# ethz-asl/laser_slam

Hardware: NVIDIA H100
Metric: ICP registrations/s (131072-pt scan vs 524288-pt map, 30 iterations) (higher is better)
Workload: dtype f32

## Files before the change

### laser_slam_b200/csrc/ls_api.cu

```cuda
#include <cstdarg>
#include <cstddef>
#include <cstdio>
#include <cstdlib>
#include <cstring>
#include <string>
#include <utility>
#include <vector>

#include "../../include/ls_b200.h"
#include "ls_kernels.cuh"

using namespace ls;

#define LS_VERSION 100

struct Workspace {
  cudaStream_t stream = nullptr;
  cudaEvent_t ev0 = nullptr, ev1 = nullptr, ev2 = nullptr, ev_launch = nullptr;
  int n_cap = 0, m_cap = 0, cells_cap = 0, tab_cap = 0, hist_cap = 0;
  BuildArrays A{};
  BuildState* bs = nullptr;
  float4* rd = nullptr;
  int* pos = nullptr;
  float4 *vq = nullptr, *vpts = nullptr;
// ... 318 lines not shown
  hp.lists.vq = w->vq;
  hp.lists.vpts = w->vpts;
  hp.lists.n = n;
  hp.work = w->work;
  hp.shard_rank = 0;
  hp.shard_count = 1;
  std::memset(&hp.link, 0, sizeof(hp.link));
  hp.T_hist = want_hist ? w->T_hist : nullptr;
  if (want_hist) {
    CU(cudaMemsetAsync(w->T_hist, 0, (size_t)prm->max_iterations * 16 * sizeof(float), w->stream));
    w->stream_dirty = true;
  }
  hp.want_matches = want_matches ? 1 : 0;
  hp.phase_ns = nullptr;
  std::memcpy(hp.T0, T0, sizeof(hp.T0));
  return LS_OK;
}

int prep_icp(ls_ctx* ctx, Workspace* w, const ls_icp_params* prm, const float4* reading_dev, int n, const float T0[16],
             bool want_matches, bool want_hist) {
  w->job_host->reading = reading_dev;
  w->job_host->n = n;
  CU(cudaMemcpyAsync(w->job_dev, w->job_host, sizeof(BuildJob), cudaMemcpyHostToDevice, w->stream));
  int rc;
  if ((rc = launch_reading_sort(ctx, w->job_dev, 1, n, resolve(prm), w->stream))) return rc;
  CU(cudaEventRecord(w->ev1, w->stream));
  CU(cudaMemsetAsync(w->work, 0, sizeof(IcpWork), w->stream));
  return fill_problem(ctx, w, prm, n, T0, want_matches, want_hist);
}

int launch_icp(ls_ctx* ctx, const ls_icp_params* prm, int batch, int n_max, bool sharded = false) {
  Workspace* w0 = ctx->ws[0];
  for (int b = 0; b < batch; ++b) ctx->probs_host[b] = ctx->ws[b]->hp;
  CU(cudaMemcpyAsync(ctx->probs_dev, ctx->probs_host, sizeof(IcpProblem) * (size_t)batch, cudaMemcpyHostToDevice, w0->stream));
  IcpParamsDev dp;
  dp.max_iterations = prm->max_iterations;
  dp.trim_ratio = prm->trim_ratio;
  dp.use_differential = prm->use_differential;
  dp.min_diff_rot = prm->min_diff_rot;
  dp.min_diff_trans = prm->min_diff_trans;
  dp.smooth_length = prm->smooth_length;
  int ctas = ctx->icp_ctas / batch;
  const int need = (n_max + 31) / 32;
  if (ctas > need) ctas = need;
  if (ctas < 1) ctas = 1;
  const IcpProblem* probs = ctx->probs_dev;
  int dynamic = batch > 1 ? 1 : 0;
  void* args[] = {(void*)&probs, (void*)&ctas, (void*)&dp, (void*)&dynamic};
  if (sharded) {
    shard_slice_kernel<<<1, 32, 0, w0->stream>>>(ctx->probs_dev, w0->job_dev, w0->hp.shard_rank, w0->hp.shard_count);
    LAUNCH_CHECK();
  }
  CU(cudaEventRecord(w0->ev_launch, w0->stream));
  CU(cudaLaunchCooperativeKernel((void*)icp_kernel, dim3(ctas * batch), dim3(kIcpThreads), args, kIcpPairBytes, w0->stream));
  ++ctx->launches;
  CU(cudaEventRecord(w0->ev2, w0->stream));
  for (int b = 0; b < batch; ++b) {
    Workspace* w = ctx->ws[b];
    constexpr size_t off = offsetof(IcpWork, T_out);
    CU(cudaMemcpyAsync(reinterpret_cast<char*>(w->h_work) + off, reinterpret_cast<const char*>(w->work) + off,
                       sizeof(IcpWork) - off, cudaMemcpyDeviceToHost, w0->stream));
    CU(cudaMemcpyAsync(w->h_grid, &w->bs->grid, sizeof(Grid), cudaMemcpyDeviceToHost, w0->stream));
  }
  return LS_OK;
}

int fetch_icp(ls_ctx* ctx, Workspace* w, int n, const float T0[16], float T_out[16], ls_icp_stats* stats,
              bool batch_timing = false) {
  const IcpWork& wk = *w->h_work;
  std::memcpy(T_out, wk.T_out, 16 * sizeof(float));
  if (stats) {
    std::memset(stats, 0, sizeof(*stats));
    stats->iterations = wk.iterations;
    stats->converged = wk.converged;
    stats->max_iter_reached = wk.max_iter_reached;
    stats->last_kept = wk.last_kept;
    stats->last_limit = wk.last_limit;
    stats->used_ratio = n > 0 ? (float)wk.last_kept / (float)n : 0.f;
    float ms = 0.f, bms = 0.f, kms = 0.f;
    const Workspace* tw = batch_timing ? ctx->ws[0] : w;
    cudaEventElapsedTime(&ms, tw->ev0, ctx->ws[0]->ev2);
    cudaEventElapsedTime(&bms, tw->ev0, tw->ev1);
    cudaEventElapsedTime(&kms, ctx->ws[0]->ev_launch, ctx->ws[0]->ev2);
    stats->device_ms = ms;
    stats->build_ms = bms;
    stats->icp_ms = kms;
    stats->grid_cells = w->h_grid->n_cells0;
    stats->grid_tables = w->h_grid->n_tab1;
    stats->grid_overflow = w->h_grid->overflow;
  }
  if (wk.status != 0) {
    std::memcpy(T_out, T0, 16 * sizeof(float));
    return fail(ctx, LS_ERR_CONVERGENCE, "ICP: no point to minimise / non-finite transformation");
  }
  return LS_OK;
}

int run_icp(ls_ctx* ctx, const ls_icp_params* prm, const float4* reading_dev, int n, const float T0[16],
            float T_out[16], ls_icp_stats* stats, int32_t* opt_ids, float* opt_d2, float* opt_T_hist) {
  Workspace* w = ctx->ws[0];
  int rc;
  if ((rc = prep_icp(ctx, w, prm, reading_dev, n, T0, opt_ids || opt_d2, opt_T_hist != nullptr))) return rc;
  if ((rc = launch_icp(ctx, prm, 1, n))) return rc;
  if (opt_ids) CU(cudaMemcpyAsync(opt_ids, w->ids, (size_t)n * sizeof(int), cudaMemcpyDeviceToHost, w->stream));
  if (opt_d2) CU(cudaMemcpyAsync(opt_d2, w->d2_out, (size_t)n * sizeof(float), cudaMemcpyDeviceToHost, w->stream));
  if (opt_T_hist)
    CU(cudaMemcpyAsync(opt_T_hist, w->T_hist, (size_t)prm->max_iterations * 16 * sizeof(float), cudaMemcpyDeviceToHost,
// ... 58 lines not shown
            cudaEventCreate(&w->ev0) == cudaSuccess && cudaEventCreate(&w->ev1) == cudaSuccess &&
            cudaEventCreate(&w->ev2) == cudaSuccess && cudaEventCreate(&w->ev_launch) == cudaSuccess &&
            cudaMalloc((void**)&w->bs, sizeof(BuildState)) == cudaSuccess &&
            cudaMallocHost((void**)&w->h_work, sizeof(IcpWork)) == cudaSuccess &&
            cudaMallocHost((void**)&w->h_grid, sizeof(Grid)) == cudaSuccess;
  if (!ok) return nullptr;
  return w;
}
void free_workspace(Workspace* w) {
  if (!w) return;
  if (w->stream) cudaStreamSynchronize(w->stream);
  void* bufs[] = {w->A.sub_pts, w->A.sub_nrm, w->A.srt_pts, w->A.srt_nrm, w->A.pkey, w->A.top, w->A.cnt0, w->A.tab1, w->A.cnt1,
                  w->A.tab1_cell, w->A.pyr, w->A.topmask, w->bs, w->rd, w->pos, w->d2,
                  w->ids, w->vq, w->vpts, w->T_hist, w->d2_out, w->A.qkey, w->A.qperm, w->A.rd_s,
                  w->A.qtab_local, w->A.qtab_total, w->A.qtop_start};
  for (void* b : bufs)
    if (b) cudaFree(b);
  if (w->h_work) cudaFreeHost(w->h_work);
  if (w->h_grid) cudaFreeHost(w->h_grid);
  if (w->ev0) cudaEventDestroy(w->ev0);
  if (w->ev1) cudaEventDestroy(w->ev1);
  if (w->ev2) cudaEventDestroy(w->ev2);
  if (w->ev_launch) cudaEventDestroy(w->ev_launch);
  if (w->stream) cudaStreamDestroy(w->stream);
  delete w;
}
int ensure_workspaces(ls_ctx* ctx, int count) {
  while ((int)ctx->ws.size() < count) {
    Workspace* w = new_workspace(ctx, (int)ctx->ws.size());
    if (!w) return fail(ctx, LS_ERR_NOMEM, "workspace allocation failed");
    ctx->ws.push_back(w);
  }
  return LS_OK;
}
}

int ls_b200_init(int device, ls_ctx** out) {
  if (!out) return LS_ERR_ARG;
  *out = nullptr;
  int count = 0;
  if (cudaGetDeviceCount(&count) != cudaSuccess || count <= 0) return LS_ERR_CUDA;
  if (device < 0 || device >= count) return LS_ERR_ARG;
  ls_ctx* ctx = new ls_ctx();
  ctx->device = device;
  auto bail = [&](int code) {
    ls_b200_destroy(ctx);
    return code;
  };
  if (cudaSetDevice(device) != cudaSuccess) return bail(LS_ERR_CUDA);
  cudaDeviceProp prop;
  if (cudaGetDeviceProperties(&prop, device) != cudaSuccess) return bail(LS_ERR_CUDA);
  if (!prop.cooperativeLaunch) return bail(LS_ERR_CUDA);
  ctx->sm_count = prop.multiProcessorCount;
  int occ = 0;
  if (cudaFuncSetAttribute(icp_kernel, cudaFuncAttributeMaxDynamicSharedMemorySize, kIcpPairBytes) != cudaSuccess ||
      cudaOccupancyMaxActiveBlocksPerMultiprocessor(&occ, icp_kernel, kIcpThreads, kIcpPairBytes) != cudaSuccess || occ < 1)
    return bail(LS_ERR_CUDA);
  ctx->icp_ctas = ctx->icp_ctas_max = occ * ctx->sm_count;
  if (cudaMalloc((void**)&ctx->probs_dev, sizeof(IcpProblem) * kMaxBatch) != cudaSuccess) return bail(LS_ERR_NOMEM);
  if (cudaMallocHost((void**)&ctx->probs_host, sizeof(IcpProblem) * kMaxBatch) != cudaSuccess) return bail(LS_ERR_NOMEM);
  if (cudaMalloc((void**)&ctx->jobs_dev, sizeof(BuildJob) * kMaxBatch) != cudaSuccess) return bail(LS_ERR_NOMEM);
  if (cudaMallocHost((void**)&ctx->jobs_host, sizeof(BuildJob) * kMaxBatch) != cudaSuccess) return bail(LS_ERR_NOMEM);
  if (cudaMalloc((void**)&ctx->work_pool, sizeof(IcpWork) * kMaxBatch) != cudaSuccess) return bail(LS_ERR_NOMEM);
  if (cudaMalloc((void**)&ctx->T0_dev, 16 * sizeof(float)) != cudaSuccess) return bail(LS_ERR_NOMEM);
  if (ensure_workspaces(ctx, 1) != LS_OK) return bail(LS_ERR_NOMEM);
  *out = ctx;
  return LS_OK;
}

void ls_b200_destroy(ls_ctx* ctx) {
  if (!ctx) return;
  cudaSetDevice(ctx->device);
  for (Workspace* w : ctx->ws) free_workspace(w);
  if (ctx->probs_dev) cudaFree(ctx->probs_dev);
  if (ctx->probs_host) cudaFreeHost(ctx->probs_host);
  if (ctx->jobs_dev) cudaFree(ctx->jobs_dev);
  if (ctx->jobs_host) cudaFreeHost(ctx->jobs_host);
  if (ctx->work_pool) cudaFree(ctx->work_pool);
  void* stage[] = {ctx->reading, ctx->ref_stage, ctx->ref_nrm_stage, ctx->nrm_raw, ctx->T0_dev};
  for (void* b : stage)
    if (b) cudaFree(b);
  ls_shard_exchange_close(ctx);
  delete ctx;
}

const char* ls_b200_last_error(const ls_ctx* ctx) { return ctx ? ctx->err.c_str() : "null context"; }
uint64_t ls_b200_launch_count(const ls_ctx* ctx) { return ctx ? ctx->launches : 0; }
int ls_b200_set_icp_cta_budget(ls_ctx* ctx, int ctas) {
  if (!ctx || ctas < 0) return LS_ERR_ARG;
  BUSY_CHECK(ctx);
  ctx->icp_ctas = (ctas == 0 || ctas > ctx->icp_ctas_max) ? ctx->icp_ctas_max : ctas;
  return LS_OK;
}
int ls_b200_icp_cta_budget(const ls_ctx* ctx) { return ctx ? ctx->icp_ctas : LS_ERR_ARG; }

void ls_icp_default_params(ls_icp_params* p) {
  if (!p) return;
  p->max_iterations = 40;
  p->trim_ratio = 0.75f;
  p->use_differential = 1;
  p->min_diff_rot = 0.001f;
  p->min_diff_trans = 0.01f;
  p->smooth_length = 4;
  p->cell_size = 0.f;
  p->leaf_split = 0;
  p->max_cells = 0;
  p->reading_sampling_prob = 1.0f;
  p->reference_normals_knn = 0;
  p->reference_sampling_ratio = 1.0f;
  p->unapplied_modules = 0;
// ... 626 lines not shown
```

### laser_slam_b200/csrc/ls_grid.cuh

```cuda
#pragma once
#include <cfloat>
#include <climits>
#include <cstring>

#include <vector_types.h>
#include <vector_functions.h>

#include "ls_math.cuh"

#define LS_FB 8
#define LS_FB3 (LS_FB * LS_FB * LS_FB)

namespace ls {

struct Entry {
  uint32_t start;
  int32_t meta;
};

struct Grid {
  float org[3];
  float H0, H1;
  float inv0, inv1;
  int dim[3];
// ... 38 lines not shown
  float d[LS_KNN_MAX];
  int id[LS_KNN_MAX];
  int k;
  float cap;
  LS_HD void reset(int kk) {
    k = kk;
    cap = INFINITY;
    for (int j = 0; j < LS_KNN_MAX; ++j) { d[j] = INFINITY; id[j] = INT_MAX; }
  }
  LS_HD float bound() const { return fminf(d[k - 1], cap); }
  LS_HD void offer(float dist, int i, int) {
    if (dist > cap || !(dist < d[k - 1] || (dist == d[k - 1] && i < id[k - 1]))) return;
    for (int j = 0; j < k; ++j)
      if (id[j] == i) return;
    int j = k - 1;
    while (j > 0 && (dist < d[j - 1] || (dist == d[j - 1] && i < id[j - 1]))) {
      d[j] = d[j - 1];
      id[j] = id[j - 1];
      --j;
    }
    d[j] = dist;
    id[j] = i;
  }
  LS_HD void offer_pt(float dist, const float4& c, int p);
};

#if defined(LS_SIM_COUNTERS) && !defined(__CUDA_ARCH__)
extern thread_local long long ls_sim_cand, ls_sim_entries, ls_sim_steps;
#define LS_CNT_CAND() (++ls_sim_cand)
#define LS_CNT_ENTRY() (++ls_sim_entries)
#define LS_CNT_STEP() (++ls_sim_steps)
#else
#define LS_CNT_CAND() ((void)0)
#define LS_CNT_ENTRY() ((void)0)
#define LS_CNT_STEP() ((void)0)
#endif

#if defined(__CUDA_ARCH__)
LS_HD float4 ld_pt(const float4* p) { return __ldg(p); }
LS_HD Entry ld_entry(const Entry* e) {
  const int2 v = __ldg(reinterpret_cast<const int2*>(e));
  Entry r;
  r.start = (uint32_t)v.x;
  r.meta = v.y;
  return r;
}
LS_HD int f2i(float f) { return __float_as_int(f); }
LS_HD float i2f(int i) { return __int_as_float(i); }
LS_HD float4 ld_state4(const float4* p) { return __ldcg(p); }
LS_HD void st_state4(float4* p, const float4 v) { __stcg(p, v); }
LS_HD unsigned long long ld_mask(const unsigned long long* p) { return __ldg(p); }
LS_HD unsigned long long ld_rows(const unsigned long long* p) { return __ldg(p); }
LS_HD int ctz64(unsigned long long m) { return __ffsll((long long)m) - 1; }
#else
LS_HD float4 ld_pt(const float4* p) { LS_CNT_CAND(); return *p; }
LS_HD Entry ld_entry(const Entry* e) { LS_CNT_ENTRY(); return *e; }
LS_HD int f2i(float f) { int i; std::memcpy(&i, &f, 4); return i; }
LS_HD float i2f(int i) { float f; std::memcpy(&f, &i, 4); return f; }
LS_HD float4 ld_state4(const float4* p) { return *p; }
LS_HD void st_state4(float4* p, const float4 v) { *p = v; }
LS_HD unsigned long long ld_mask(const unsigned long long* p) { LS_CNT_ENTRY(); return *p; }
LS_HD unsigned long long ld_rows(const unsigned long long* p) { return *p; }
LS_HD int ctz64(unsigned long long m) { return __builtin_ctzll(m); }
#endif

LS_HD int coord_top(float v, float o, float inv, int n) {
  float t = floorf((v - o) * inv);
  t = fminf(fmaxf(t, 0.0f), (float)(n - 1));
  return (int)t;
}
LS_HD int coord_sub(float v, float lo, float inv) {
  float t = floorf((v - lo) * inv);
  t = fminf(fmaxf(t, 0.0f), (float)(LS_FB - 1));
  return (int)t;
}
LS_HD float cell_lo(float o, int c, float H) { return o + (float)c * H; }

LS_HD float gap(float q, float lo, float hi, float m) {
  const float a = (lo - m) - q;
  const float b = q - (hi + m);
  return fmaxf(0.0f, fmaxf(a, b));
}

#define LS_SHRINK 0.999999f

LS_HD float ball_radius(float best_d2, float margin) { return sqrtf(best_d2) * 1.000001f + margin; }

LS_HD void Best::offer_pt(float d, const float4& c, int p) { offer(d, f2i(c.w), p); }
LS_HD void TopK::offer_pt(float dist, const float4& c, int p) { offer(dist, f2i(c.w), p); }
template <class Acc>
LS_HD void consider_pt(const float4 p, int pos, float qx, float qy, float qz, Acc& b) {
  b.offer_pt(dist2(qx, qy, qz, p.x, p.y, p.z), p, pos);
}
template <class Acc>
LS_HD void consider(const float4* pts, int pos, float qx, float qy, float qz, Acc& b) {
  consider_pt(ld_pt(pts + pos), pos, qx, qy, qz, b);
}

template <class Acc>
LS_HD void scan_range(const float4* pts, uint32_t a, uint32_t e, float qx, float qy, float qz, Acc& b) {
  uint32_t pos = a;
  for (; pos + 4 <= e; pos += 4) {
    LS_CNT_STEP();
    const float4 p0 = ld_pt(pts + pos), p1 = ld_pt(pts + pos + 1), p2 = ld_pt(pts + pos + 2), p3 = ld_pt(pts + pos + 3);
    consider_pt(p0, (int)pos, qx, qy, qz, b);
    consider_pt(p1, (int)pos + 1, qx, qy, qz, b);
    consider_pt(p2, (int)pos + 2, qx, qy, qz, b);
    consider_pt(p3, (int)pos + 3, qx, qy, qz, b);
  }
  if (pos < e) LS_CNT_STEP();
  for (; pos < e; ++pos) consider(pts, (int)pos, qx, qy, qz, b);
}

template <class Acc>
LS_HD void visit_fine(const Grid& g, const Entry* tab, unsigned long long rows, float lox, float loy, float loz,
                      const float4* pts, float qx, float qy, float qz, Acc& b) {
// ... 178 lines not shown
#ifndef LS_VL_GATE
#define LS_VL_GATE 1.0f
#endif
struct VLists {
  float4* vq;
  float4* vpts;
  int n;
};

struct Collector {
  float r2;
  int cnt;
  float4* out;
  int stride;
  LS_HD float bound() const { return r2; }
  LS_HD void offer_pt(float d, const float4& c, int p) {
    if (d <= r2) {
      if (cnt < LS_VK) st_state4(out + (size_t)cnt * stride, make_float4(c.x, c.y, c.z, i2f(p)));
      else r2 = -1.0f;
      ++cnt;
    }
  }
};

LS_HD bool vlist_query(const VLists& L, const float4* pts, int i, const float4 v, const float4 c0, float qx, float qy,
                       float qz, float cap_d2, Best& b, float4& cbest) {
  const unsigned int bits = (unsigned int)f2i(v.w);
  if (bits == 0u) return false;
  const int cnt = (int)(bits & 15u);
  const float Rv = i2f((int)(bits & ~15u));
  const float Rc = Rv * 0.999996f - sqrtf(dist2(qx, qy, qz, v.x, v.y, v.z)) * 1.000004f;
  if (!(Rc > 0.0f)) return false;
  b.d2 = cap_d2;
  b.idx = INT_MAX;
  b.pos = -1;
  for (int k = 0; k < cnt; ++k) {
    const float4 c = k == 0 ? c0 : ld_state4(L.vpts + (size_t)k * L.n + i);
    const float d = dist2(qx, qy, qz, c.x, c.y, c.z);
    const int cpos = f2i(c.w);
    if (d < b.d2) {
      b.d2 = d;
      b.pos = cpos;
      cbest = c;
    } else if (d == b.d2) {
      if (b.pos < 0 || f2i(ld_pt(pts + cpos).w) < f2i(ld_pt(pts + b.pos).w)) {
        b.pos = cpos;
        cbest = c;
      }
    }
  }
  return b.d2 * 1.00001f <= Rc * Rc;
}

LS_HD void vlist_build(const Grid& g, const GridView& v, const VLists& L, int i, float qx, float qy, float qz, bool found,
                       float found_d2, float cap_d2, float motion) {
  float Rv;
  if (found) {
    const float want = sqrtf(found_d2);
    const float margin = fmaxf(want * LS_VL_REL, LS_VL_ABS) + 1e-4f;
    if (!(motion * LS_VL_GATE <= margin)) return;
    Rv = want + fminf(margin, fmaxf(0.002f, LS_VL_SKIN * motion));
  } else {
    const float want = sqrtf(cap_d2);
    if (!(motion <= want * 0.125f)) return;
    Rv = want * 1.05f + fminf(want * 0.25f, fmaxf(0.002f, 4.0f * motion));
  }
  if (!(Rv < 3.0e38f)) return;
  Collector c;
  c.r2 = Rv * Rv;
  c.cnt = 0;
  c.out = L.vpts + i;
  c.stride = L.n;
  ball_query(g, v, qx, qy, qz, c);
  float4 head = make_float4(qx, qy, qz, 0.0f);
  if (c.cnt <= LS_VK) head.w = i2f((int)((((unsigned int)f2i(Rv * 0.9999999f)) & ~15u) | (unsigned int)c.cnt));
  st_state4(L.vq + i, head);
}

LS_HDN void knn_search(const Grid& g, const GridView& v, float qx, float qy, float qz, int k, TopK& t) {
  t.reset(k);
  if (g.m <= 0) return;
  const float extent = g.H0 * (float)(g.dim[0] + g.dim[1] + g.dim[2]) + 1.0f;
  float R = g.H1;
  for (int round = 0; round < 64; ++round) {
    t.cap = R * R;
    ball_query(g, v, qx, qy, qz, t);
    if (t.d[k - 1] <= t.cap) break;
    if (R > extent + fabsf(qx - g.org[0]) + fabsf(qy - g.org[1]) + fabsf(qz - g.org[2])) break;
    R = R * 2.0f;
  }
}

LS_HD int top_index(const Grid& g, float x, float y, float z) {
  const int cx = coord_top(x, g.org[0], g.inv0, g.dim[0]);
  const int cy = coord_top(y, g.org[1], g.inv0, g.dim[1]);
  const int cz = coord_top(z, g.org[2], g.inv0, g.dim[2]);
  return (cz * g.dim[1] + cy) * g.dim[0] + cx;
}
LS_HD void top_origin(const Grid& g, int c0, float& lox, float& loy, float& loz) {
  const int cx = c0 % g.dim[0];
  const int cy = (c0 / g.dim[0]) % g.dim[1];
  const int cz = c0 / (g.dim[0] * g.dim[1]);
  lox = cell_lo(g.org[0], cx, g.H0);
  loy = cell_lo(g.org[1], cy, g.H0);
  loz = cell_lo(g.org[2], cz, g.H0);
}
LS_HD int sub_index(float x, float y, float z, float lox, float loy, float loz, float inv) {
  return (coord_sub(z, loz, inv) * LS_FB + coord_sub(y, loy, inv)) * LS_FB + coord_sub(x, lox, inv);
}

LS_HDN void grid_setup(Grid& g, const float* lo, const float* hi, float cell_size, int max_cells, int leaf_split,
                       int m) {
  float H = cell_size > 0.f ? cell_size : 2.0f;
  float ext[3], emax = 0.f, oabs = 0.f;
  for (int a = 0; a < 3; ++a) {
    ext[a] = hi[a] - lo[a];
    if (!(ext[a] >= 0.f)) ext[a] = 0.f;
    emax = fmaxf(emax, ext[a]);
    oabs = fmaxf(oabs, fmaxf(fabsf(lo[a]), fabsf(hi[a])));
  }
  for (int it = 0; it < 40; ++it) {
    double cells = 1.0;
    for (int a = 0; a < 3; ++a) cells *= floor((double)ext[a] / (double)H) + 1.0;
    if (cells <= (double)max_cells) break;
    H = H * 2.0f;
  }
  g.H0 = H;
  g.H1 = H / (float)LS_FB;
  g.inv0 = 1.0f / g.H0;
  g.inv1 = 1.0f / g.H1;
  int n = 1;
  for (int a = 0; a < 3; ++a) {
    g.org[a] = lo[a];
    int d = (int)floorf(ext[a] * g.inv0) + 1;
    if (d < 1) d = 1;
    g.dim[a] = d;
    n *= d;
  }
  g.n_cells0 = n;
  g.margin = (oabs + emax + H) * 1.9073486328125e-06f;
  g.m = m;
  g.leaf_split = leaf_split > 0 ? leaf_split : 32;
  g.n_tab1 = 0;
  g.overflow = 0;
// ... 15 lines not shown
```

### laser_slam_b200/csrc/ls_kernels.cuh

```cuda
#pragma once
#include <cuda_runtime.h>
#include <cooperative_groups.h>

#include "ls_grid.cuh"

namespace ls {

constexpr int kMaxParts = 16;
constexpr int kScanTile = 4096;
constexpr int kScanThreads = 512;
constexpr int kIcpThreads = 512;
constexpr int kIcpCtasPerSm = 1024 / kIcpThreads;
constexpr int kMaxSmooth = 15;
constexpr uint32_t kTag1 = 1u << 31, kKeyMask = (1u << 31) - 1u;

struct Parts {
  int n_parts;
  int offset[kMaxParts + 1];
  const float4* pts[kMaxParts];
  const float4* nrm[kMaxParts];
  float T[kMaxParts][16];
  int identity[kMaxParts];
};

// ... 957 lines not shown

__device__ __forceinline__ void push_pairs(const IcpProblem& P, PairQueue& Q, int sign, float sx, float sy, float sz,
                                           const float4 q, int pos) {
  const unsigned int m = __ballot_sync(0xffffffffu, sign != 0);
  if (m == 0u) return;
  if (sign) {
    float f[6], e;
    residual_terms(sx, sy, sz, q, __ldg(P.nrm + pos), f, e);
    const int slot = (Q.head + Q.cnt + __popc(m & ((1u << (threadIdx.x & 31)) - 1u))) & (kPairSlots - 1);
    float4* r = reinterpret_cast<float4*>(Q.recs + slot * 8);
    r[0] = make_float4(f[0], f[1], f[2], f[3]);
    r[1] = make_float4(f[4], f[5], e, (float)sign);
  }
  Q.cnt += __popc(m);
  __syncwarp();
  if (Q.cnt >= 32) {
    Q.acc = consume_pairs(Q.recs, Q.head, 32, Q.acc);
    Q.head = (Q.head + 32) & (kPairSlots - 1);
    Q.cnt -= 32;
    __syncwarp();
  }
}

__device__ __forceinline__ void drain_pairs(PairQueue& Q, unsigned long long* slab) {
  if (Q.cnt > 0) {
    Q.acc = consume_pairs(Q.recs, Q.head, Q.cnt, Q.acc);
    Q.head = (Q.head + Q.cnt) & (kPairSlots - 1);
    Q.cnt = 0;
  }
  const int lane = threadIdx.x & 31;
  if (lane < 28) slab[lane] = (unsigned long long)Q.acc;
  Q.acc = 0ll;
  __syncwarp();
}

__device__ __noinline__ void phase_a_search(const Grid* gp, const IcpProblem* Pp, const float* T_iter, const float* T_prev,
                                            int i, float cap, SelHists* H, unsigned int pred_bin1, unsigned int pred_pref12) {
  if (i < 0) return;
  const Grid& g = *gp;
  const IcpProblem& P = *Pp;
  const float4 r = __ldg(P.rd + i);
  float sx, sy, sz;
  xform_point(T_iter, r.x, r.y, r.z, sx, sy, sz);
  const int warm = __ldcg(P.pos + i);
  const Best b = nn_search(g, P.view, sx, sy, sz, warm, cap);
  phase_a_record(P, i, b, H, pred_bin1, pred_pref12);
  if (T_prev) {
    float px, py, pz;
    xform_point(T_prev, r.x, r.y, r.z, px, py, pz);
    vlist_build(g, P.view, P.lists, i, sx, sy, sz, b.pos >= 0, b.d2, cap, sqrtf(dist2(sx, sy, sz, px, py, pz)));
  }
}

__device__ __forceinline__ void push_searched(const IcpProblem& P, PairQueue& Q, const float* T_iter, int j, float acc_limit) {
  if (!(acc_limit >= 0.0f)) return;
  float d = INFINITY;
  if (j >= 0) d = __ldcg(P.d2 + j);
  const bool keep = d <= acc_limit;
  if (__ballot_sync(0xffffffffu, keep) == 0u) return;
  float4 q = make_float4(0.f, 0.f, 0.f, 0.f);
  float sx = 0.f, sy = 0.f, sz = 0.f;
  int pos = -1;
  if (keep) {
    pos = __ldcg(P.pos + j);
    const float4 r = __ldg(P.rd + j);
    xform_point(T_iter, r.x, r.y, r.z, sx, sy, sz);
    q = __ldg(P.view.pts + pos);
  }
  push_pairs(P, Q, keep ? 1 : 0, sx, sy, sz, q, pos);
}

__device__ __noinline__ void final_match(const Grid* gp, const IcpProblem* Pp, const float* T, int i) {
  if (i < 0) return;
  const IcpProblem& P = *Pp;
  const float4 r = __ldg(P.rd + i);
  float sx, sy, sz;
  xform_point(T, r.x, r.y, r.z, sx, sy, sz);
  const Best b = nn_search(*gp, P.view, sx, sy, sz, __ldcg(P.pos + i), INFINITY);
  const uint32_t orig = __ldg(P.qperm + i);
  P.d2_out[orig] = b.d2;
  P.ids[orig] = b.idx;
}

__device__ __forceinline__ void flush_slabs(unsigned long long (*acc_w)[28], unsigned long long* gacc) {
  __syncthreads();
  if (threadIdx.x < 28) {
    unsigned long long t = 0ull;
#pragma unroll
    for (int w = 0; w < kIcpThreads / 32; ++w) t += acc_w[w][threadIdx.x];
    if (t != 0ull) atomicAdd(&gacc[threadIdx.x], t);
  }
  __syncthreads();
}

__device__ __forceinline__ void flush_hist(const unsigned int* hs, int nbins, unsigned int* gh) {
  for (int k = threadIdx.x; k < nbins; k += kIcpThreads) {
    const unsigned int v = hs[k];
    if (v) atomicAdd(&gh[k], v);
  }
}

__global__ void __launch_bounds__(kIcpThreads, kIcpCtasPerSm)
icp_kernel(const IcpProblem* __restrict__ probs, int ctas_per_problem, IcpParamsDev prm, int dynamic) {
  const int pi = blockIdx.x / ctas_per_problem;
  const int cta = blockIdx.x - pi * ctas_per_problem;
  const IcpProblem& P = probs[pi];
  IcpWork* W = P.work;
  const bool xg = P.shard_count > 1;
  IcpWork* X = xg ? P.link.slots + P.shard_rank : W;
  const IcpWork* S0 = xg ? P.link.slots : W;
  const int n_slots = xg ? P.shard_count : 1;
  const unsigned int G = (unsigned int)ctas_per_problem;
  unsigned int xepoch = 0;
  const int tid = threadIdx.x, lane = tid & 31;

  __shared__ Grid g;
  __shared__ float T_iter[16], T_last[16];
  __shared__ SelHists hs;
  __shared__ unsigned long long acc_w[kIcpThreads / 32][28];
  __shared__ SelectOut sel;
  __shared__ unsigned int ws[kIcpThreads / 32];
  __shared__ double qh[kMaxSmooth + 2][4];
  __shared__ double th[kMaxSmooth + 2][3];
  __shared__ int flag_stop, flag_status;
  __shared__ int miss_buf[kIcpThreads / 32][64];
  extern __shared__ __align__(16) float pair_buf[];

  if (tid == 0) {
    g = P.bs->grid;
    for (int i = 0; i < 16; ++i) T_iter[i] = (i % 5 == 0) ? 1.f : 0.f;
    quat_from_T(T_iter, qh[0]);
    th[0][0] = th[0][1] = th[0][2] = 0.0;
    flag_stop = 0;
    flag_status = 0;
  }
  __syncthreads();
  PairQueue Q;
  Q.recs = pair_buf + (tid >> 5) * (kPairSlots * 8);
  Q.head = 0;
  Q.cnt = 0;
  Q.acc = 0ll;

  const int n = P.n;
  int chunk = (n + (int)G - 1) / (int)G;
  chunk = (chunk + 31) & ~31;
  const int q_begin = min(n, cta * chunk), q_end = min(n, q_begin + chunk);

  for (int i = q_begin + tid; i < q_end; i += kIcpThreads) {
    __stcg(P.pos + i, -1);
    __stcg(P.lists.vq + i, make_float4(0.f, 0.f, 0.f, 0.f));
  }

  float cap = 0.04f;
  int redo = 0;
// ... 17 lines not shown
    __syncthreads();
    {
      const float* T_prev = iter >= 1 ? T_last : nullptr;
      int* mq = miss_buf[tid >> 5];
      int n_miss = 0;
      int next = q_begin + (tid & ~31);
      for (;;) {
        int base;
        if (dynamic) {
          unsigned int bb = 0;
          if (lane == 0) bb = atomicAdd(&W->qctr[par], 32u);
          bb = __shfl_sync(0xffffffffu, bb, 0);
          if (bb >= (unsigned int)n) break;
          base = (int)bb;
        } else {
          if (next >= q_end) break;
          base = next;
          next += kIcpThreads;
        }
        const int i = base + lane;
        bool valid = i < (dynamic ? n : q_end);
        if (redo && valid) valid = !(__ldcg(P.d2 + i) < INFINITY);
        bool hit = false;
        Best b;
        b.d2 = INFINITY; b.idx = INT_MAX; b.pos = -1;
        float4 c = make_float4(0.f, 0.f, 0.f, 0.f);
        float sx = 0.f, sy = 0.f, sz = 0.f;
        if (valid) {
          const float4 r = __ldg(P.rd + i);
          const float4 v = __ldcg(P.lists.vq + i);
          const float4 c0 = __ldcg(P.lists.vpts + i);
          xform_point(T_iter, r.x, r.y, r.z, sx, sy, sz);
          hit = vlist_query(P.lists, P.view.pts, i, v, c0, sx, sy, sz, cap, b, c);
          if (hit) phase_a_record(P, i, b, &hs, pred_bin1, pred_pref12);
        }
        push_pairs(P, Q, (hit && b.pos >= 0 && b.d2 <= acc_limit) ? 1 : 0, sx, sy, sz, c, b.pos);
        const unsigned int mm = __ballot_sync(0xffffffffu, valid && !hit);
        if (mm) {
          if (valid && !hit) mq[n_miss + __popc(mm & ((1u << lane) - 1u))] = i;
          n_miss += __popc(mm);
          __syncwarp();
          if (n_miss >= 32) {
            n_miss -= 32;
            const int j = mq[n_miss + lane];
            __syncwarp();
            phase_a_search(&g, &P, T_iter, T_prev, j, cap, &hs, pred_bin1, pred_pref12);
            push_searched(P, Q, T_iter, j, acc_limit);
          }
        }
      }
      if (n_miss > 0) {
        __syncwarp();
        const int j = lane < n_miss ? mq[lane] : -1;
        phase_a_search(&g, &P, T_iter, T_prev, j, cap, &hs, pred_bin1, pred_pref12);
        __syncwarp();
        push_searched(P, Q, T_iter, j, acc_limit);
      }
    }
    drain_pairs(Q, acc_w[tid >> 5]);
    flush_slabs(acc_w, X->acc[par]);
    flush_hist(hs.h1, 1024, X->hist[par][0]);
    if (pred_bin1 != kNoPrediction) {
      flush_hist(hs.h2, 2048, X->hist[par][3]);
      flush_hist(hs.h3, 1024, X->hist[par][4]);
    }
    {
      const int hb = kHistOff + par * 5 * 2048;
      const bool pr = pred_bin1 != kNoPrediction;
      meet(hb, 1024, hb + 3 * 2048, pr ? 2048 : 0, hb + 4 * 2048, pr ? 1024 : 0);
    }
    LS_STAMP(1);

    block_select(S0->hist[par][0], 1024, 0u, true, prm.trim_ratio, &sel, ws, n_slots);
    if (sel.total == 0u) {
      if (tid == 0) { flag_status = 1; if (cta == 0) W->fail_code = 1; }
      __syncthreads();
      break;
    }
    if (sel.bin >= 1020u) {
      if (!(cap < INFINITY)) {
        if (tid == 0) { flag_status = 1; if (cta == 0) W->fail_code = 1; }
        __syncthreads();
        break;
      }
      cap = cap < 64.0f ? cap * 4.0f : INFINITY;
      ++redo;
      meet(0, 0, 0, 0, 0, 0);
      if (cta == 0 && tid == 0) {
        X->hist[par][0][1020] = 0u;
        W->qctr[par] = 0u;
      }
      problem_barrier(&X->barrier, G, epoch);
      continue;
    }
    const unsigned int bin1 = sel.bin, rem1 = sel.rem;
    if (cta == 0) {
      unsigned int* h = &X->hist[par ^ 1][0][0];
      for (int k = tid; k < 5 * 2048; k += kIcpThreads) h[k] = 0u;
      if (tid < 32) X->acc[par ^ 1][tid] = 0ull;
    }
    if (cta == 0 && tid == 0) W->qctr[par ^ 1] = 0u;
    const bool spec2 = bin1 == pred_bin1;
    if (!spec2) {
      for (int k = tid; k < 2048; k += kIcpThreads) hs.h2[k] = 0u;
      __syncthreads();
      for (int i = q_begin + tid; i < q_end; i += kIcpThreads) {
        const unsigned int key = __float_as_uint(__ldcg(P.d2 + i));
// ... 152 lines not shown
```

Before: 901.2.

## Use cooperative lane groups for tail nearest-neighbor searches in partial warps

When a warp's leftover miss queue holds few queries (at most 8), each query is now spread across a group of 4 or 8 lanes. The lanes in a group split the grid cells, sub-cells and candidate points of the ball query and reduce the best match or verlet list with shuffles. This targets the idle lanes that the per-thread search leaves during small tail batches. The kernel is templated on this path and only used for single-problem launches. The cost is extra shuffle and scan overhead, a second kernel instance, and an occupancy taken as the minimum of the two variants.

```diff
diff --git a/laser_slam_b200/csrc/ls_api.cu b/laser_slam_b200/csrc/ls_api.cu
--- a/laser_slam_b200/csrc/ls_api.cu
+++ b/laser_slam_b200/csrc/ls_api.cu
@@ -394,7 +394,8 @@
     LAUNCH_CHECK();
   }
   CU(cudaEventRecord(w0->ev_launch, w0->stream));
-  CU(cudaLaunchCooperativeKernel((void*)icp_kernel, dim3(ctas * batch), dim3(kIcpThreads), args, kIcpPairBytes, w0->stream));
+  void* const kern = dynamic ? (void*)icp_kernel<false> : (void*)icp_kernel<true>;
+  CU(cudaLaunchCooperativeKernel(kern, dim3(ctas * batch), dim3(kIcpThreads), args, kIcpPairBytes, w0->stream));
   ++ctx->launches;
   CU(cudaEventRecord(w0->ev2, w0->stream));
   for (int b = 0; b < batch; ++b) {
@@ -559,10 +560,14 @@
   if (cudaGetDeviceProperties(&prop, device) != cudaSuccess) return bail(LS_ERR_CUDA);
   if (!prop.cooperativeLaunch) return bail(LS_ERR_CUDA);
   ctx->sm_count = prop.multiProcessorCount;
-  int occ = 0;
-  if (cudaFuncSetAttribute(icp_kernel, cudaFuncAttributeMaxDynamicSharedMemorySize, kIcpPairBytes) != cudaSuccess ||
-      cudaOccupancyMaxActiveBlocksPerMultiprocessor(&occ, icp_kernel, kIcpThreads, kIcpPairBytes) != cudaSuccess || occ < 1)
+  int occ = 0, occ1 = 0;
+  if (cudaFuncSetAttribute(icp_kernel<false>, cudaFuncAttributeMaxDynamicSharedMemorySize, kIcpPairBytes) != cudaSuccess ||
+      cudaFuncSetAttribute(icp_kernel<true>, cudaFuncAttributeMaxDynamicSharedMemorySize, kIcpPairBytes) != cudaSuccess ||
+      cudaOccupancyMaxActiveBlocksPerMultiprocessor(&occ, icp_kernel<false>, kIcpThreads, kIcpPairBytes) != cudaSuccess ||
+      cudaOccupancyMaxActiveBlocksPerMultiprocessor(&occ1, icp_kernel<true>, kIcpThreads, kIcpPairBytes) != cudaSuccess)
     return bail(LS_ERR_CUDA);
+  if (occ1 < occ) occ = occ1;
+  if (occ < 1) return bail(LS_ERR_CUDA);
   ctx->icp_ctas = ctx->icp_ctas_max = occ * ctx->sm_count;
   if (cudaMalloc((void**)&ctx->probs_dev, sizeof(IcpProblem) * kMaxBatch) != cudaSuccess) return bail(LS_ERR_NOMEM);
   if (cudaMallocHost((void**)&ctx->probs_host, sizeof(IcpProblem) * kMaxBatch) != cudaSuccess) return bail(LS_ERR_NOMEM);
diff --git a/laser_slam_b200/csrc/ls_grid.cuh b/laser_slam_b200/csrc/ls_grid.cuh
--- a/laser_slam_b200/csrc/ls_grid.cuh
+++ b/laser_slam_b200/csrc/ls_grid.cuh
@@ -114,6 +114,7 @@
 LS_HD unsigned long long ld_mask(const unsigned long long* p) { return __ldg(p); }
 LS_HD unsigned long long ld_rows(const unsigned long long* p) { return __ldg(p); }
 LS_HD int ctz64(unsigned long long m) { return __ffsll((long long)m) - 1; }
+LS_HD int popc64(unsigned long long m) { return __popcll(m); }
 #else
 LS_HD float4 ld_pt(const float4* p) { LS_CNT_CAND(); return *p; }
 LS_HD Entry ld_entry(const Entry* e) { LS_CNT_ENTRY(); return *e; }
@@ -124,6 +125,7 @@
 LS_HD unsigned long long ld_mask(const unsigned long long* p) { LS_CNT_ENTRY(); return *p; }
 LS_HD unsigned long long ld_rows(const unsigned long long* p) { return *p; }
 LS_HD int ctz64(unsigned long long m) { return __builtin_ctzll(m); }
+LS_HD int popc64(unsigned long long m) { return __builtin_popcountll(m); }
 #endif
 
 LS_HD int coord_top(float v, float o, float inv, int n) {
@@ -408,29 +410,55 @@
   return b.d2 * 1.00001f <= Rc * Rc;
 }
 
-LS_HD void vlist_build(const Grid& g, const GridView& v, const VLists& L, int i, float qx, float qy, float qz, bool found,
-                       float found_d2, float cap_d2, float motion) {
+LS_HD float vlist_radius(bool found, float found_d2, float cap_d2, float motion) {
   float Rv;
   if (found) {
     const float want = sqrtf(found_d2);
     const float margin = fmaxf(want * LS_VL_REL, LS_VL_ABS) + 1e-4f;
-    if (!(motion * LS_VL_GATE <= margin)) return;
+    if (!(motion * LS_VL_GATE <= margin)) return 0.0f;
     Rv = want + fminf(margin, fmaxf(0.002f, LS_VL_SKIN * motion));
   } else {
     const float want = sqrtf(cap_d2);
-    if (!(motion <= want * 0.125f)) return;
+    if (!(motion <= want * 0.125f)) return 0.0f;
     Rv = want * 1.05f + fminf(want * 0.25f, fmaxf(0.002f, 4.0f * motion));
   }
-  if (!(Rv < 3.0e38f)) return;
+  return Rv < 3.0e38f ? Rv : 0.0f;
+}
+
+LS_HD float4 vlist_head(float qx, float qy, float qz, float Rv, int cnt) {
+  float4 head = make_float4(qx, qy, qz, 0.0f);
+  if (cnt <= LS_VK) head.w = i2f((int)((((unsigned int)f2i(Rv * 0.9999999f)) & ~15u) | (unsigned int)cnt));
+  return head;
+}
+
+LS_HD void vlist_build(const Grid& g, const GridView& v, const VLists& L, int i, float qx, float qy, float qz, bool found,
+                       float found_d2, float cap_d2, float motion) {
+  const float Rv = vlist_radius(found, found_d2, cap_d2, motion);
+  if (!(Rv > 0.0f)) return;
   Collector c;
   c.r2 = Rv * Rv;
   c.cnt = 0;
   c.out = L.vpts + i;
   c.stride = L.n;
   ball_query(g, v, qx, qy, qz, c);
-  float4 head = make_float4(qx, qy, qz, 0.0f);
-  if (c.cnt <= LS_VK) head.w = i2f((int)((((unsigned int)f2i(Rv * 0.9999999f)) & ~15u) | (unsigned int)c.cnt));
-  st_state4(L.vq + i, head);
+  st_state4(L.vq + i, vlist_head(qx, qy, qz, Rv, c.cnt));
+}
+
+LS_HD int ball_cells(const Grid& g, float qx, float qy, float qz, float r2) {
+  const float R = ball_radius(r2, g.margin);
+  const int nx = coord_top(qx + R, g.org[0], g.inv0, g.dim[0]) - coord_top(qx - R, g.org[0], g.inv0, g.dim[0]) + 1;
+  const int ny = coord_top(qy + R, g.org[1], g.inv0, g.dim[1]) - coord_top(qy - R, g.org[1], g.inv0, g.dim[1]) + 1;
+  const int nz = coord_top(qz + R, g.org[2], g.inv0, g.dim[2]) - coord_top(qz - R, g.org[2], g.inv0, g.dim[2]) + 1;
+  return nx * ny * nz;
+}
+
+LS_HD int nth_bit64(unsigned long long m, int k) {
+  int pos = 0;
+  for (int w = 32; w >= 1; w >>= 1) {
+    const int c = popc64(m & ((1ull << w) - 1ull));
+    if (k >= c) { k -= c; m >>= w; pos += w; }
+  }
+  return pos;
 }
 
 LS_HDN void knn_search(const Grid& g, const GridView& v, float qx, float qy, float qz, int k, TopK& t) {
@@ -446,6 +474,169 @@
     R = R * 2.0f;
   }
 }
+
+#if defined(__CUDACC__)
+template <int L>
+__device__ __forceinline__ int group_scan(int v, int& total) {
+  const int l = threadIdx.x & (L - 1);
+  int s = v;
+#pragma unroll
+  for (int o = 1; o < L; o <<= 1) {
+    const int t = __shfl_up_sync(0xffffffffu, s, o, L);
+    if (l >= o) s += t;
+  }
+  total = __shfl_sync(0xffffffffu, s, L - 1, L);
+  return s - v;
+}
+template <int L>
+__device__ __forceinline__ int group_owner(int off, int t) {
+  int o = 0;
+#pragma unroll
+  for (int s = L / 2; s >= 1; s >>= 1)
+    if (__shfl_sync(0xffffffffu, off, o + s, L) <= t) o += s;
+  return o;
+}
+
+template <int L, class Acc>
+__device__ __forceinline__ void group_ball(const Grid& g, const GridView& v, bool on, float qx, float qy, float qz, Acc& a) {
+  const int l = threadIdx.x & (L - 1);
+  const float R = ball_radius(a.bound(), g.margin);
+  const int x0 = coord_top(qx - R, g.org[0], g.inv0, g.dim[0]), nx = coord_top(qx + R, g.org[0], g.inv0, g.dim[0]) - x0 + 1;
+  const int y0 = coord_top(qy - R, g.org[1], g.inv0, g.dim[1]), ny = coord_top(qy + R, g.org[1], g.inv0, g.dim[1]) - y0 + 1;
+  const int z0 = coord_top(qz - R, g.org[2], g.inv0, g.dim[2]), nz = coord_top(qz + R, g.org[2], g.inv0, g.dim[2]) - z0 + 1;
+  const int n_cell = on ? nx * ny * nz : 0;
+  const int cell_rounds = __reduce_max_sync(0xffffffffu, n_cell);
+  for (int cb = 0; cb < cell_rounds; cb += L) {
+    const int c = cb + l;
+    Entry e{0u, 0};
+    unsigned long long rows = 0ull;
+    float cy = 0.f, cz = 0.f;
+    int fx = 0;
+    int n_item = 0;
+    if (c < n_cell) {
+      const int x = x0 + c % nx, y = y0 + (c / nx) % ny, z = z0 + c / (nx * ny);
+      const float cx = cell_lo(g.org[0], x, g.H0);
+      cy = cell_lo(g.org[1], y, g.H0);
+      cz = cell_lo(g.org[2], z, g.H0);
+      const float gz = gap(qz, cz, cell_lo(g.org[2], z + 1, g.H0), g.margin);
+      const float gy = gap(qy, cy, cell_lo(g.org[1], y + 1, g.H0), g.margin);
+      const float gx = gap(qx, cx, cell_lo(g.org[0], x + 1, g.H0), g.margin);
+      const float lb = gx * gx + (gy * gy + gz * gz);
+      if (!(lb * LS_SHRINK > a.bound())) {
+        const size_t ci = ((size_t)z * g.dim[1] + y) * g.dim[0] + x;
+        e = ld_entry(v.top + ci);
+        rows = ld_rows(v.topmask + ci);
+        if (e.meta > 0) {
+          n_item = 1;
+        } else if (e.meta < 0) {
+          const float R1 = ball_radius(a.bound(), g.margin);
+          fx = coord_sub(qx - R1, cx, g.inv1) | coord_sub(qx + R1, cx, g.inv1) << 8;
+          const int fy0 = coord_sub(qy - R1, cy, g.inv1), fy1 = coord_sub(qy + R1, cy, g.inv1);
+          const int fz0 = coord_sub(qz - R1, cz, g.inv1), fz1 = coord_sub(qz + R1, cz, g.inv1);
+          const unsigned long long ym = (unsigned long long)((2u << fy1) - (1u << fy0));
+          unsigned long long in = 0ull;
+          for (int zz = fz0; zz <= fz1; ++zz) in |= ym << (zz * LS_FB);
+          rows &= in;
+          n_item = popc64(rows);
+        }
+      }
+    }
+    int n_items;
+    const int ioff = group_scan<L>(n_item, n_items);
+    const int item_rounds = __reduce_max_sync(0xffffffffu, n_items);
+    for (int ib = 0; ib < item_rounds; ib += L) {
+      const int t = ib + l;
+      const int o = group_owner<L>(ioff, t);
+      const int k = t - __shfl_sync(0xffffffffu, ioff, o, L);
+      const uint32_t o_start = __shfl_sync(0xffffffffu, e.start, o, L);
+      const int o_meta = __shfl_sync(0xffffffffu, e.meta, o, L);
+      const unsigned long long o_rows =
+          (unsigned long long)__shfl_sync(0xffffffffu, (unsigned int)rows, o, L) |
+          (unsigned long long)__shfl_sync(0xffffffffu, (unsigned int)(rows >> 32), o, L) << 32;
+      const float o_cy = __shfl_sync(0xffffffffu, cy, o, L), o_cz = __shfl_sync(0xffffffffu, cz, o, L);
+      const int o_fx = __shfl_sync(0xffffffffu, fx, o, L);
+      uint32_t r0 = 0u, r1 = 0u;
+      if (t < n_items) {
+        if (o_meta > 0) {
+          r0 = o_start;
+          r1 = o_start + (uint32_t)o_meta;
+        } else {
+          const int bit = nth_bit64(o_rows, k);
+          const int z = bit / LS_FB, y = bit % LS_FB;
+          const float gz = gap(qz, cell_lo(o_cz, z, g.H1), cell_lo(o_cz, z + 1, g.H1), g.margin);
+          const float gy = gap(qy, cell_lo(o_cy, y, g.H1), cell_lo(o_cy, y + 1, g.H1), g.margin);
+          const float lb = gy * gy + gz * gz;
+          if (!(lb * LS_SHRINK > a.bound())) {
+            const Entry* row = v.tab1 + (size_t)(~o_meta) * LS_FB3 + (z * LS_FB + y) * LS_FB;
+            const Entry e0 = ld_entry(row + (o_fx & 255));
+            const Entry e1 = ld_entry(row + (o_fx >> 8));
+            r0 = e0.start;
+            r1 = e1.start + (uint32_t)e1.meta;
+          }
+        }
+      }
+      int n_cand;
+      const int coff = group_scan<L>((int)(r1 - r0), n_cand);
+      const int cand_rounds = __reduce_max_sync(0xffffffffu, n_cand);
+      for (int kb = 0; kb < cand_rounds; kb += 4 * L) {
+        int p[4];
+#pragma unroll
+        for (int u = 0; u < 4; ++u) {
+          const int tt = kb + u * L + l;
+          const int oo = group_owner<L>(coff, tt);
+          const int at = (int)__shfl_sync(0xffffffffu, r0, oo, L) + (tt - __shfl_sync(0xffffffffu, coff, oo, L));
+          p[u] = tt < n_cand ? at : -1;
+        }
+        float4 pt[4];
+#pragma unroll
+        for (int u = 0; u < 4; ++u) pt[u] = p[u] >= 0 ? ld_pt(v.pts + p[u]) : make_float4(0.f, 0.f, 0.f, 0.f);
+#pragma unroll
+        for (int u = 0; u < 4; ++u) a.offer(p[u] >= 0, dist2(qx, qy, qz, pt[u].x, pt[u].y, pt[u].z), pt[u], p[u]);
+        a.sync();
+      }
+    }
+  }
+}
+
+template <int L>
+struct GroupBest {
+  Best b;
+  __device__ float bound() const { return b.d2; }
+  __device__ void offer(bool take, float d, const float4& c, int p) {
+    if (take) b.offer_pt(d, c, p);
+  }
+  __device__ void sync() {
+#pragma unroll
+    for (int o = 1; o < L; o <<= 1) {
+      const float d = __shfl_xor_sync(0xffffffffu, b.d2, o, L);
+      const int i = __shfl_xor_sync(0xffffffffu, b.idx, o, L);
+      const int p = __shfl_xor_sync(0xffffffffu, b.pos, o, L);
+      b.offer(d, i, p);
+    }
+  }
+};
+
+template <int L>
+struct GroupCollect {
+  float r2;
+  int cnt;
+  float4* out;
+  int stride;
+  __device__ float bound() const { return r2; }
+  __device__ void offer(bool take, float d, const float4& c, int p) {
+    take = take && d <= r2;
+    const int lane = threadIdx.x & 31;
+    const unsigned int gm = (__ballot_sync(0xffffffffu, take) >> (lane & ~(L - 1))) & (0xffffffffu >> (32 - L));
+    if (take) {
+      const int slot = cnt + __popc(gm & ((1u << (lane & (L - 1))) - 1u));
+      if (slot < LS_VK) st_state4(out + (size_t)slot * stride, make_float4(c.x, c.y, c.z, i2f(p)));
+    }
+    cnt += __popc(gm);
+    if (cnt > LS_VK) r2 = -1.0f;
+  }
+  __device__ void sync() {}
+};
+#endif
 
 LS_HD int top_index(const Grid& g, float x, float y, float z) {
   const int cx = coord_top(x, g.org[0], g.inv0, g.dim[0]);
diff --git a/laser_slam_b200/csrc/ls_kernels.cuh b/laser_slam_b200/csrc/ls_kernels.cuh
--- a/laser_slam_b200/csrc/ls_kernels.cuh
+++ b/laser_slam_b200/csrc/ls_kernels.cuh
@@ -1033,6 +1033,81 @@
   }
 }
 
+template <int L>
+__device__ __noinline__ void phase_a_group(const Grid* gp, const IcpProblem* Pp, const float* T_iter, const float* T_prev,
+                                           int i, float cap, SelHists* H, unsigned int pred_bin1, unsigned int pred_pref12) {
+  constexpr int kGroups = 32 / L;
+  const Grid& g = *gp;
+  const IcpProblem& P = *Pp;
+  const int lane = threadIdx.x & 31;
+  const int home = (lane % kGroups) * L;
+  float4 r = make_float4(0.f, 0.f, 0.f, 0.f);
+  float sx = 0.f, sy = 0.f, sz = 0.f;
+  Best b;
+  b.d2 = cap;
+  b.idx = INT_MAX;
+  b.pos = -1;
+  bool grp = false;
+  if (i >= 0 && g.m > 0) {
+    r = __ldg(P.rd + i);
+    xform_point(T_iter, r.x, r.y, r.z, sx, sy, sz);
+    const int warm = __ldcg(P.pos + i);
+    if (warm >= 0) consider(P.view.pts, warm, sx, sy, sz, b);
+    else seed_query(g, P.view, sx, sy, sz, b);
+    if (ball_cells(g, sx, sy, sz, b.bound()) > 27) ball_query(g, P.view, sx, sy, sz, b);
+    else grp = true;
+  }
+  for (int rd = 0; rd < L; ++rd) {
+    const int src = rd * kGroups + lane / L;
+    const bool on = __shfl_sync(0xffffffffu, grp, src);
+    if (!__any_sync(0xffffffffu, on)) continue;
+    GroupBest<L> a;
+    a.b.d2 = __shfl_sync(0xffffffffu, b.d2, src);
+    a.b.idx = __shfl_sync(0xffffffffu, b.idx, src);
+    a.b.pos = __shfl_sync(0xffffffffu, b.pos, src);
+    group_ball<L>(g, P.view, on, __shfl_sync(0xffffffffu, sx, src), __shfl_sync(0xffffffffu, sy, src),
+                            __shfl_sync(0xffffffffu, sz, src), a);
+    const float d = __shfl_sync(0xffffffffu, a.b.d2, home);
+    const int id = __shfl_sync(0xffffffffu, a.b.idx, home), ps = __shfl_sync(0xffffffffu, a.b.pos, home);
+    if (grp && lane / kGroups == rd) {
+      b.d2 = d;
+      b.idx = id;
+      b.pos = ps;
+    }
+  }
+  if (b.pos < 0) { b.idx = -1; b.d2 = INFINITY; }
+  if (i >= 0) phase_a_record(P, i, b, H, pred_bin1, pred_pref12);
+  if (!T_prev) return;
+  float Rv = 0.f;
+  grp = false;
+  if (i >= 0 && g.m > 0) {
+    float px, py, pz;
+    xform_point(T_prev, r.x, r.y, r.z, px, py, pz);
+    const float motion = sqrtf(dist2(sx, sy, sz, px, py, pz));
+    Rv = vlist_radius(b.pos >= 0, b.d2, cap, motion);
+    if (Rv > 0.f && ball_cells(g, sx, sy, sz, Rv * Rv) > 27) {
+      vlist_build(g, P.view, P.lists, i, sx, sy, sz, b.pos >= 0, b.d2, cap, motion);
+      Rv = 0.f;
+    }
+    grp = Rv > 0.f;
+  }
+  for (int rd = 0; rd < L; ++rd) {
+    const int src = rd * kGroups + lane / L;
+    const bool on = __shfl_sync(0xffffffffu, grp, src);
+    if (!__any_sync(0xffffffffu, on)) continue;
+    const float R = __shfl_sync(0xffffffffu, Rv, src);
+    GroupCollect<L> c;
+    c.r2 = R * R;
+    c.cnt = 0;
+    c.out = P.lists.vpts + __shfl_sync(0xffffffffu, i, src);
+    c.stride = P.lists.n;
+    group_ball<L>(g, P.view, on, __shfl_sync(0xffffffffu, sx, src), __shfl_sync(0xffffffffu, sy, src),
+                            __shfl_sync(0xffffffffu, sz, src), c);
+    const int cnt = __shfl_sync(0xffffffffu, c.cnt, home);
+    if (grp && lane / kGroups == rd) st_state4(P.lists.vq + i, vlist_head(sx, sy, sz, Rv, cnt));
+  }
+}
+
 __device__ __forceinline__ void push_searched(const IcpProblem& P, PairQueue& Q, const float* T_iter, int j, float acc_limit) {
   if (!(acc_limit >= 0.0f)) return;
   float d = INFINITY;
@@ -1081,6 +1156,7 @@
   }
 }
 
+template <bool kGroupTail>
 __global__ void __launch_bounds__(kIcpThreads, kIcpCtasPerSm)
 icp_kernel(const IcpProblem* __restrict__ probs, int ctas_per_problem, IcpParamsDev prm, int dynamic) {
   const int pi = blockIdx.x / ctas_per_problem;
@@ -1204,7 +1280,13 @@
       if (n_miss > 0) {
         __syncwarp();
         const int j = lane < n_miss ? mq[lane] : -1;
-        phase_a_search(&g, &P, T_iter, T_prev, j, cap, &hs, pred_bin1, pred_pref12);
+        if constexpr (kGroupTail) {
+          if (n_miss <= 4) phase_a_group<8>(&g, &P, T_iter, T_prev, j, cap, &hs, pred_bin1, pred_pref12);
+          else if (n_miss <= 8) phase_a_group<4>(&g, &P, T_iter, T_prev, j, cap, &hs, pred_bin1, pred_pref12);
+          else phase_a_search(&g, &P, T_iter, T_prev, j, cap, &hs, pred_bin1, pred_pref12);
+        } else {
+          phase_a_search(&g, &P, T_iter, T_prev, j, cap, &hs, pred_bin1, pred_pref12);
+        }
         __syncwarp();
         push_searched(P, Q, T_iter, j, acc_limit);
       }
```

Result: faster. 916.3 (median of 6 runs) (+1.7%).
